# mit-acl/roman

Hardware: AMD Instinct MI355X
Metric: submap-pair alignments/sec + p50 latency at n=m=200 objects, d=512 (higher is better)
Workload: dtype f64 (fixed-point SpMV sums); 1 GPU; config 3: batch of 256 submap pairs per GPU, n=200 m=200 d=512, method=semanticgrav (xyz + 512-d descriptors + gravity prior); p50 latency measured on config 2 (single pair); pairs_per_call=256, n=200, m=200, d=512, method=semanticgrav, batches_in_flight=3

## Files before the change

### roman_amd/csrc/kernels.hip.h

```cpp
#pragma once
#include <hip/hip_cooperative_groups.h>
#include <hip/hip_runtime.h>
#include <stdint.h>
#include <type_traits>
#include "../../include/roman_hip.h"

namespace roman {

constexpr int WAVE = 64;
constexpr int STREAM_MAXL = 3072;

struct DevParams {
    roman_params_t p;
    double sig2;
    double sin_unc;
    double x_eps;
    double x_mindist;
    int32_t single;
    int32_t gravity;
    int32_t F;
    int32_t max_compact;
    int32_t gmode;
    int32_t diag_one;
    int32_t keep_all;
// ... 779 lines not shown
#pragma unroll
    for (int m = 0; m < MAXB; ++m) {
        if (m < cnt) {
            const int e = e0 + m, bx = e / nby, by = e - bx * nby;
            const int col = j0 + 16 * by + lr;
            const double nb = nrm[16 * T + 16 * by + lr];
#pragma unroll
            for (int r = 0; r < 4; ++r) {
                const int row = i0 + 16 * bx + kq + 4 * r;
                const double na = nrm[16 * bx + kq + 4 * r];
                if (row < iEnd && col < jEnd)
                    cosPool[pd.cosOff + (int64_t)row * pd.n2 + col] = D.pruned ? acc[m][r] : ((na > 0.0 && nb > 0.0) ? acc[m][r] / (na * nb) : 0.0);
            }
        }
    }
}

constexpr int CSEL_ROWS = 512;
constexpr int CSEL_MAXN = 256;
constexpr int CSEL_CAP = 4096;
constexpr int CSEL_NPT = CSEL_CAP / 1024;
constexpr int CSEL_P1 = 256 + 16;
constexpr int CSEL_P2 = 128 + 16;
constexpr int CSEL_MP = 11;
constexpr int CSEL_STAGE = CSEL_ROWS * CSEL_P1;
static_assert(CSEL_ROWS * CSEL_P2 + 2 * CSEL_CAP * 4 <= CSEL_STAGE, "pass 2 fits where the tile was");
constexpr int CSEL_LDS = CSEL_STAGE + CSEL_ROWS * 8 + 2 * 260 * 4;
typedef __bf16 bf16x8_t __attribute__((ext_vector_type(8)));
typedef float f32x4_t __attribute__((ext_vector_type(4)));
struct __attribute__((packed, aligned(8))) d8u_t { double v[8]; };

__device__ __forceinline__ bool csel_unsafe(double n) { return !(n >= 0x1p-40 && n <= 0x1p40); }

__global__ void __launch_bounds__(1024) k_cos_sel(DevParams D, int B, const ProbDesc* __restrict__ probs, const double* __restrict__ feats,
                                                  double* __restrict__ cosPool, int32_t* __restrict__ dense ,
                                                  double thr )
{
    extern __shared__ __attribute__((aligned(16))) unsigned char smem[];
    unsigned char* stage = smem;
    double* nrm = reinterpret_cast<double*>(smem + CSEL_STAGE);
    uint32_t* U = reinterpret_cast<uint32_t*>(smem + CSEL_ROWS * CSEL_P2);
    uint32_t* S = U + CSEL_CAP;
    int* hist = reinterpret_cast<int*>(nrm + CSEL_ROWS);
    int* cur = hist + 260;
    const int b = blockIdx.x;
    if (b >= B) return;
    const ProbDesc pd = probs[b];
    const int tid = threadIdx.x, lane = tid & 63, w = uni_i(tid >> 6);
    const int n1 = pd.n1, n2 = pd.n2;
    if (n1 <= 0 || n2 <= 0) { if (tid == 0) dense[b] = 0; return; }
    const int nb1 = (n1 + 15) >> 4, nb2 = (n2 + 15) >> 4, RB = 16 * nb1, nblk = nb1 * nb2, rowsTot = RB + 16 * nb2;
    if (n1 > CSEL_MAXN || n2 > CSEL_MAXN || nblk > 16 * CSEL_MP) { if (tid == 0) dense[b] = 1; return; }
    const int Fc = D.p.cos_feature_dim, coff = D.p.point_dim + D.p.ratio_feature_dim;
    if (tid < 260) hist[tid] = 0;
    const double* base1 = feats + pd.off1 * D.F + coff;
    const double* base2 = feats + pd.off2 * D.F + coff;

    constexpr int KT = 128, G1 = 4;
    const int nt = rowsTot >> 4;
    const int NG8 = ((nt + 2 * G1 - 1) / (2 * G1)) * 2;
    const int NSF = Fc / KT;
    uint32_t slotLo, slotHi;
    {
        const int R = w + 16 * min(lane, nt - 1);
        const bool isA = R < RB;
        const int idx = min(isA ? R : R - RB, (isA ? n1 : n2) - 1);
        const uint64_t pa = reinterpret_cast<uint64_t>((isA ? base1 : base2) + (int64_t)idx * D.F);
        slotLo = (uint32_t)pa; slotHi = (uint32_t)(pa >> 32);
    }
    auto slot_ptr = [&](int t) -> const double* {
        const uint64_t lo = (uint32_t)__builtin_amdgcn_readlane((int)slotLo, t), hi = (uint32_t)__builtin_amdgcn_readlane((int)slotHi, t);
        return reinterpret_cast<const double*>((hi << 32) | lo);
    };
    auto load_group = [&](dbl2_t (&x)[G1], int st, int g) {
        const int ko = st * KT + 2 * lane;
#pragma unroll
        for (int j = 0; j < G1; ++j) {
            const d2u_t tv = *reinterpret_cast<const d2u_t*>(slot_ptr(G1 * g + j) + ko);
            x[j] = dbl2_t{tv.v[0], tv.v[1]};
        }
        __builtin_amdgcn_sched_barrier(0);
    };
    auto load_group_ragged = [&](dbl2_t (&x)[G1], int st, int g) {
// ... 45 lines not shown
            }
        }
    };
    {
        dbl2_t xa[G1], xb[G1];
        if (NSF > 0) { load_group(xa, 0, 0); load_group(xb, 0, 1); }
        for (int st = 0; st < NSF; ++st) {
            for (int g = 0; g < NG8; g += 2) {
                const int gn = g + 2 < NG8 ? g + 2 : 0, stn = g + 2 < NG8 ? st : min(st + 1, NSF - 1);
                stage_group(xa, g);
                load_group(xa, stn, gn);
                stage_group(xb, g + 1);
                load_group(xb, stn, gn + 1);
            }
            __syncthreads();
            multiply();
            __syncthreads();
        }
        if (NSF * KT < Fc) {
            for (int g = 0; g < NG8; ++g) { load_group_ragged(xa, NSF, g); stage_group(xa, g); }
            __syncthreads();
            multiply();
            __syncthreads();
        }
    }
#pragma unroll
    for (int m = 0; m < 2; ++m)
        if (w + 16 * m < nt) {
            const int r4 = lane & 3;
            const float v = r4 == 0 ? accD[m][0] : r4 == 1 ? accD[m][1] : r4 == 2 ? accD[m][2] : accD[m][3];
            if (((lane & 15) >> 2) == (lane >> 4)) nrm[16 * (w + 16 * m) + (lane & 15)] = sqrt((double)v);
        }
    __syncthreads();

    const unsigned long long lt = (1ull << lane) - 1ull;
#pragma unroll
    for (int m = 0; m < CSEL_MP; ++m)
        if (m < cntP) {
            const int e = e0 + m, bx = e / nb2, by = e - bx * nb2;
            const int j = 16 * by + (lane & 15);
            const double nbv = nrm[RB + j];
#pragma unroll
            for (int rr = 0; rr < 4; ++rr) {
                const int i = 16 * bx + 4 * (lane >> 4) + rr;
                const double na = nrm[i];
                const bool ok = i < n1 && j < n2;
                const double cv = (double)acc[m][rr] / (na * nbv);
                const bool cand = ok && (csel_unsafe(na) || csel_unsafe(nbv) || !(cv < thr));
                if (ok && !cand) cosPool[pd.cosOff + (int64_t)i * n2 + j] = cv;
                const unsigned long long bm = __ballot(cand);
                if (bm) {
                    int base = 0;
                    if (lane == 0) base = atomicAdd(&hist[256], __popcll(bm));
                    base = __shfl(base, 0);
                    if (cand) {
                        const int slot = base + __popcll(bm & lt);
                        if (slot < CSEL_CAP) U[slot] = (uint32_t)i | ((uint32_t)j << 16);
                        atomicAdd(&hist[i], 1);
                    }
                }
            }
        }
    __syncthreads();
    const int nc = hist[256];
    if (nc > CSEL_CAP) { if (tid == 0) dense[b] = 1; return; }
    if (tid == 0) dense[b] = 0;
    if (nc == 0) return;
    if (w == 0) {
        const int c0 = hist[4 * lane], c1 = hist[4 * lane + 1], c2 = hist[4 * lane + 2], c3 = hist[4 * lane + 3];
        int incl = c0 + c1 + c2 + c3;
#pragma unroll
        for (int d = 1; d < 64; d <<= 1) { const int t = __shfl_up(incl, d); if (lane >= d) incl += t; }
        const int ex = incl - (c0 + c1 + c2 + c3);
        cur[4 * lane] = ex; cur[4 * lane + 1] = ex + c0; cur[4 * lane + 2] = ex + c0 + c1; cur[4 * lane + 3] = ex + c0 + c1 + c2;
    }
    __syncthreads();
    for (int q = tid; q < nc; q += 1024) { const uint32_t v = U[q]; S[atomicAdd(&cur[v & 0xffffu], 1)] = v; }
    __syncthreads();

    constexpr int NQ = CSEL_ROWS / 128;
    const int pp = lane & 7, laneRow = 8 * w + (lane >> 3);
    uint32_t rofs[NQ];
#pragma unroll
    for (int q = 0; q < NQ; ++q) {
        const int R = min(128 * q + laneRow, rowsTot - 1);
        const bool isA = R < RB;
        const int idx = min(isA ? R : R - RB, (isA ? n1 : n2) - 1);
        rofs[q] = (uint32_t)((((isA ? pd.off1 : pd.off2) + idx) * D.F + coff + 2 * pp) * 8);
    }
    const char* pool = reinterpret_cast<const char*>(feats);
    auto load16 = [&](dbl2_t (&x)[NQ], int k0) {
#pragma unroll
        for (int q = 0; q < NQ; ++q) { const d2u_t t = *reinterpret_cast<const d2u_t*>(pool + (rofs[q] + (uint32_t)(8 * k0))); x[q] = dbl2_t{t.v[0], t.v[1]}; }
    };
    auto load16_ragged = [&](dbl2_t (&x)[NQ], int k0) {
        const int k = k0 + 2 * pp;
#pragma unroll
        for (int q = 0; q < NQ; ++q) { const double* rb = reinterpret_cast<const double*>(pool + rofs[q]); x[q] = dbl2_t{k < Fc ? rb[k0] : 0.0, k + 1 < Fc ? rb[k0 + 1] : 0.0}; }
    };
    uint32_t my[CSEL_NPT]; double dot[CSEL_NPT];
    const int cnt2 = nc > tid ? (nc - tid + 1023) >> 10 : 0;
#pragma unroll
    for (int m = 0; m < CSEL_NPT; ++m) { my[m] = m < cnt2 ? S[m * 1024 + tid] : 0u; dot[m] = 0.0; }
    const int rN = tid >> 1, hN = tid & 1;
    double s0 = 0.0, s1 = 0.0;
    auto put16 = [&](const dbl2_t (&x)[NQ]) {
#pragma unroll
        for (int q = 0; q < NQ; ++q)
            *reinterpret_cast<dbl2_t*>(stage + (128 * q + laneRow) * CSEL_P2 + 16 * pp) = x[q];
    };
    auto compute = [&](int s, auto fullChunk) {
// ... 26 lines not shown
#pragma unroll
                        for (int g = 0; g < 4; ++g) if (4 * g + 2 * tp + 1 < kleft) d = fma(av[g].y, bv[g].y, d);
                    }
                }
                dot[m] = d;
            }
    };
    {
        const int NCF = Fc >> 4;
        dbl2_t ya[NQ], yb[NQ];
        if (NCF > 0) { load16(ya, 0); load16(yb, 16 * min(1, NCF - 1)); }
        for (int s = 0; s < NCF; s += 2) {
            put16(ya);
            __syncthreads();
            load16(ya, 16 * min(s + 2, NCF - 1));
            compute(s, std::true_type{});
            __syncthreads();
            if (s + 1 < NCF) {
                put16(yb);
                __syncthreads();
                load16(yb, 16 * min(s + 3, NCF - 1));
                compute(s + 1, std::true_type{});
                __syncthreads();
            }
        }
        if (NCF * 16 < Fc) {
            load16_ragged(ya, 16 * NCF);
            put16(ya);
            __syncthreads();
            compute(NCF, std::false_type{});
            __syncthreads();
        }
    }
    {
        const double p = s0 + s1, q = __shfl_xor(p, 1);
        if (hN == 0) nrm[rN] = sqrt(p + q);
    }
    __syncthreads();
#pragma unroll
    for (int m = 0; m < CSEL_NPT; ++m)
        if (m < cnt2) {
            const int i = (int)(my[m] & 0xffffu), j = (int)(my[m] >> 16);
            const double na = nrm[i], nbv = nrm[RB + j];
            cosPool[pd.cosOff + (int64_t)i * n2 + j] = (na > 0.0 && nbv > 0.0) ? dot[m] / (na * nbv) : 0.0;
        }
}

__global__ void __launch_bounds__(1024) k_tables(DevParams D, const ProbDesc* __restrict__ probs,
                                                 const double* __restrict__ feats,
                                                 double* __restrict__ tabPool, int RB ,
                                                 uint16_t* __restrict__ qtabPool )
{
    extern __shared__ __attribute__((aligned(16))) double s_xyz[];
    const ProbDesc pd = probs[blockIdx.z];
    const int which = blockIdx.y;
    const int n = which == 0 ? pd.n1 : pd.n2;
    const int r0 = blockIdx.x * RB;
    if (r0 >= n) return;
    const int64_t base = which == 0 ? pd.off1 : pd.off2;
    const int pdim = D.p.point_dim;
    for (int t = threadIdx.x; t < n * 3; t += blockDim.x) {
        const int o = t / 3, c = t - o * 3;
        s_xyz[t] = (c < pdim) ? feats[(base + o) * D.F + c] : 0.0;
    }
    __syncthreads();
    double* tab = tabPool + pd.tabOff + (which == 0 ? 0 : (int64_t)pd.n1 * pd.n1);
    const int nq = (n + 3) & ~3;
    uint16_t* qtab = qtabPool ? qtabPool + 4 * (int64_t)pd.qtabOff4 + (which == 0 ? 0 : (int64_t)pd.n1 * ((pd.n1 + 3) & ~3)) : nullptr;
    const int lane = threadIdx.x & 63, w = threadIdx.x >> 6, nw = blockDim.x >> 6;
    for (int rr = w; rr < RB; rr += nw) {
        const int a = r0 + rr;
        if (a >= n) break;
        const double ax = s_xyz[3 * a], ay = s_xyz[3 * a + 1], az = s_xyz[3 * a + 2];
        for (int b = lane; b < n; b += WAVE) {
            const double dx = ax - s_xyz[3 * b], dy = ay - s_xyz[3 * b + 1], dz = az - s_xyz[3 * b + 2];
            const double h2 = dx * dx + dy * dy;
            const double l2 = h2 + dz * dz;
            const bool bad = (a == b) || (D.p.mindist > 0.0 && l2 < D.x_mindist);
            const double v = (D.gmode == 1 || D.gmode == 2) ? sqrt(h2) : sqrt(l2);
            tab[(int64_t)a * n + b] = bad ? d_nan() : v;
            if (qtab) qtab[(int64_t)a * nq + b] = (uint16_t)(uint32_t)__builtin_fmin((bad ? d_nan() : v) * D.pre_invw, 32767.0);
        }
    }
}

constexpr int LIVE_CHUNK = 4096;

template <int PHASE>
__global__ void __launch_bounds__(256) k_live(DevParams D, const ProbDesc* __restrict__ probs,
                                              ProbState* __restrict__ st,
                                              const double* __restrict__ feats,
                                              const int32_t* __restrict__ assoc,
                                              const double* __restrict__ cosPool,
                                              double* __restrict__ qS, int32_t* __restrict__ qP ,
                                              int32_t* __restrict__ segCnt, int maxChunks,
                                              int32_t* __restrict__ lp, int32_t* __restrict__ li,
                                              int32_t* __restrict__ lj, double* __restrict__ ls, double* __restrict__ ld,
                                              double* __restrict__ lza, double* __restrict__ lzb)
{
    __shared__ int cbase[2];
    __shared__ uint16_t survQ[PHASE == 0 ? 4 : 1][PHASE == 0 ? LIVE_CHUNK / 4 : 1];
    const int b = blockIdx.y, c = blockIdx.x;
    const ProbDesc pd = probs[b];
    const int tid = threadIdx.x, w = tid >> 6, lane = tid & 63;
    const int nA = pd.nA;
    const int nChunks = (nA + LIVE_CHUNK - 1) / LIVE_CHUNK;
    if (c >= nChunks && !(PHASE == 1 && c == 0)) return;
    constexpr int SEG = LIVE_CHUNK / 4;
    constexpr int NIT = SEG / WAVE;
    const int p_beg = min(nA, c * LIVE_CHUNK + w * SEG), p_end = min(nA, p_beg + SEG);
    const int Fc = D.p.cos_feature_dim;
    const int64_t lo = pd.liveOff;
    int32_t* sc = segCnt + (int64_t)b * maxChunks * 4;
    const unsigned long long lt = (1ull << lane) - 1ull;

    if (PHASE == 0) {
        const int pdm = D.p.point_dim;
        auto full_score = [&](int p) {
            int i, j;
            decode_assoc(pd, assoc, p, i, j);
            const double cosv = (Fc > 0) ? cosPool[pd.cosOff + (int64_t)i * pd.n2 + j] : 0.0;
            const double* fi = feats + (pd.off1 + i) * D.F + pdm; const double* fj = feats + (pd.off2 + j) * D.F + pdm;
            return single_score(D, [&](int f) { return fi[f]; }, [&](int f) { return fj[f]; }, cosv);
        };
        int nlive = 0;
        auto emit = [&](bool valid, int p, double s) {
            const bool live = valid && (s > 0.0 || D.keep_all);
            const unsigned long long m = __ballot(live);
            if (live) { const int k = p_beg + nlive + __popcll(m & lt); qP[lo + k] = p; qS[lo + k] = s; }
            nlive += __popcll(m);
        };
        if (D.single && Fc > 0 && !D.keep_all) {
            uint16_t* q = survQ[w];
            const double cden = D.p.cosine_max - D.p.cosine_min;
            int ns = 0;
// ... 20 lines not shown
            __builtin_amdgcn_wave_barrier();
            __builtin_amdgcn_fence(__ATOMIC_ACQUIRE, "wavefront");
            for (int k0 = 0; k0 < ns; k0 += WAVE) {
                const int k = k0 + lane;
                const int p = p_beg + (int)q[min(k, max(ns - 1, 0))];
                emit(k < ns, p, k < ns ? full_score(p) : 0.0);
            }
        } else {
            for (int p0 = p_beg; p0 < p_end; p0 += WAVE) {
                const int p = p0 + lane;
                emit(p < p_end, p, (p < p_end && D.single) ? full_score(p) : 1.0);
            }
        }
        if (lane == 0) sc[c * 4 + w] = nlive;
        return;
    }

    if (w == 0) {
        int front = 0, total = 0;
        for (int k0 = 0; k0 < nChunks * 4; k0 += WAVE) {
            const int k = k0 + lane;
            const int v = k < nChunks * 4 ? sc[k] : 0;
            int f = k < c * 4 ? v : 0, t = v;
            for (int off = 32; off > 0; off >>= 1) { f += __shfl_xor(f, off); t += __shfl_xor(t, off); }
            front += f; total += t;
        }
        if (lane == 0) { cbase[0] = front; cbase[1] = total; }
    }
    __syncthreads();
    const bool all_live = D.pruned && cbase[1] == 0 && nA > 0;
    const int Ltot = all_live ? nA : cbase[1];
    if (c == 0 && tid == 0) {
        st[b].L = Ltot; st[b].nnzUpper = 0ull;
        st[b].kind = (Ltot <= D.stream_maxL && D.p.maxiniters >= 1 && D.p.maxlsiters >= 1) ? 0 : (D.allow_fallback ? 1 : 2);
    }
    if (c >= nChunks) return;
    int base = cbase[0];
    for (int k = 0; k < w; ++k) base += sc[c * 4 + k];
    const int n = all_live ? p_end - p_beg : sc[c * 4 + w];
    if (all_live) base = p_beg;
    const bool has_z = D.p.point_dim == 3;
    for (int k0 = 0; k0 < n; k0 += WAVE) {
        const int k = k0 + lane;
        if (k < n) {
            const int p = all_live ? p_beg + k : qP[lo + p_beg + k];
            const double s = all_live ? 1.0 : qS[lo + p_beg + k];
            int i, j;
            decode_assoc(pd, assoc, p, i, j);
            const int pos = base + k;
            lp[lo + pos] = p; li[lo + pos] = i; lj[lo + pos] = j; ls[lo + pos] = s;
            ld[lo + pos] = D.diag_one ? 1.0 : s;
            lza[lo + pos] = has_z ? feats[(pd.off1 + i) * D.F + 2] : 0.0;
            lzb[lo + pos] = has_z ? feats[(pd.off2 + j) * D.F + 2] : 0.0;
        }
    }
}

template <class T>
__device__ __forceinline__ T block_excl_scan(T v, T* sh, T& total)
{
    const int lane = threadIdx.x & 63, w = threadIdx.x >> 6, nw = blockDim.x >> 6;
    T inc = v;
    for (int off = 1; off < WAVE; off <<= 1) { const T t = __shfl_up(inc, off); if (lane >= off) inc += t; }
    __syncthreads();
    if (lane == WAVE - 1) sh[w] = inc;
    __syncthreads();
    T base = 0, tot = 0;
// ... 4374 lines not shown
```

### roman_amd/csrc/roman_hip.hip

```cpp
#include <hip/hip_runtime.h>
#include <algorithm>
#include <cmath>
#include <cstdarg>
#include <cstdio>
#include <cstdlib>
#include <cstring>
#include <new>
#include <string>
#include <vector>

#include "kernels.hip.h"

using namespace roman;

namespace {

thread_local std::string g_last_error;

struct DevBuf {
    void* p = nullptr; size_t cap = 0;
    hipError_t ensure(size_t bytes) {
        if (bytes <= cap) return hipSuccess;
        if (p) { hipError_t e = hipFree(p); p = nullptr; cap = 0; if (e != hipSuccess) return e; }
        size_t want = bytes + bytes / 4 + 256;
// ... 269 lines not shown
        heurMaxL = std::max(heurMaxL, (int)capL);
        heurMask += capL * std::ceil(capL / 64.0);
        heurNnz += capL * std::min(capL, 96.0);
    }
    if (H.valid) {
        S->expectMaxL = prunes ? (int)std::min(S->maxA, std::ceil(H.rMaxL * S->maxA * 1.15) + 64.0) : (int)S->maxA;
        S->capMaskWords = (long long)(prunes ? H.rMask * S->maskBound * 1.3 + 4096.0 : S->maskBound);
        S->capNnz = (long long)(H.rNnz * S->sumA * 1.3 + 65536.0);
        S->capList = (long long)(H.rList * S->sumA * 1.3 + 65536.0);
    } else {
        S->expectMaxL = heurMaxL; S->capMaskWords = (long long)heurMask; S->capNnz = (long long)heurNnz + 65536;
        S->capList = (long long)(2.5 * heurNnz) + 65536;
    }
    S->capMaskWords = std::max<long long>(S->capMaskWords, 64);
    const char* tcap = getenv("ROMAN_TEST_CAPNNZ");
    if (tcap && !H.valid) S->capNnz = atoll(tcap);
}

int may_fallback(const DevParams& D, const std::vector<ProbDesc>& hd);

struct BatchOut { int32_t kmax; int32_t* assoc_out; int32_t* n_assoc_out; double* T_out; int32_t* status_out; roman_stats_t* stats_out; };

int make_solve_out(roman_ctx* c, int B, int64_t sumA, const BatchOut& out, SolveOut* O)
{
    const size_t R1 = (size_t)std::max<int64_t>(sumA, 1);
    HIPCHK(c, WS.uOut.ensure(sizeof(double) * R1)); HIPCHK(c, WS.nodesOrig.ensure(sizeof(int32_t) * R1));
    HIPCHK(c, WS.nSel.ensure(sizeof(int32_t) * (size_t)B));
    O->assoc_out = out.assoc_out; O->n_assoc_out = out.n_assoc_out; O->T_out = out.T_out; O->status_out = out.status_out; O->stats_out = out.stats_out; O->kmax = out.kmax;
    O->nodesOrig = WS.nodesOrig.as<int32_t>(); O->nSel = WS.nSel.as<int32_t>(); O->uOut = WS.uOut.as<double>();
    O->dbg = nullptr;
    return ROMAN_OK;
}

static hipError_t launch_cos_sel(roman_ctx* c, hipStream_t stream, const DevParams& D, int B, int maxN1, int maxN2, const ProbDesc* dP, const double* feats, double* cosPool,
                                 int32_t* dense, bool approx)
{
    hipError_t e = dyn_lds(c, reinterpret_cast<const void*>(k_cos_sel), (size_t)CSEL_LDS);
    if (e != hipSuccess) return e;
    const double thr = approx ? INFINITY : D.p.cosine_min - 0x1p-6;
    hipLaunchKernelGGL(k_cos_sel, dim3((unsigned)B), dim3(1024), (size_t)CSEL_LDS, stream, D, B, dP, feats, cosPool, dense, thr);
    e = hipGetLastError();
    if (e != hipSuccess) return e;
    constexpr int TD = 5;
    using CD = CosDeal<TD>;
    const int Gd = CD::tiles(maxN1) * CD::tiles(maxN2);
    e = dyn_lds(c, reinterpret_cast<const void*>(k_cos_deal<TD, 0>), (size_t)CD::LDS);
    if (e != hipSuccess) return e;
    hipLaunchKernelGGL((k_cos_deal<TD, 0>), dim3((unsigned)(B >= 8 ? Gd * ((B + 7) / 8) * 8 : Gd * B)), dim3(256), (size_t)CD::LDS, stream, D, B, Gd, dP, feats, cosPool, (const int32_t*)dense);
    return hipGetLastError();
}
static bool cos_sel_applies(const roman_ctx* c, const DevParams& D, int B, int maxN1, int maxN2, int64_t poolRows)
{
    if (!D.single || D.pruned || !(D.p.cosine_max > D.p.cosine_min) || !std::isfinite(D.p.cosine_min) || !std::isfinite(D.p.cosine_max)) return false;
    if (maxN1 > CSEL_MAXN || maxN2 > CSEL_MAXN || maxN1 <= 0 || maxN2 <= 0) return false;
    if (poolRows * (int64_t)D.F * 8 >= (1LL << 32)) return false;
    const char* env = getenv("ROMAN_COS_SEL");
    if (env && env[0]) return env[0] == '1';
    if (2 * B < c->num_cu || D.p.cos_feature_dim < 64 || std::max(maxN1, maxN2) < 64) return false;
    roman_ctx::Hist& H = const_cast<roman_ctx*>(c)->hist;
    if (H.cosSeen && H.cosDenseFrac > 0.25) {
        if (++H.cosSkipped < 64) return false;
        H.cosSkipped = 0;
    }
    return true;
}


static int sort_eq_max()
{
    const char* e = getenv("ROMAN_SORT_EQMAX");
    return (e && e[0]) ? std::max(0, atoi(e)) : 512;
}

static hipError_t launch_cos(roman_ctx* c, hipStream_t stream, const DevParams& D, int B, int maxN1, int maxN2, const ProbDesc* dP, const double* feats, double* cosPool)
{
// ... 26 lines not shown
        const int nbx = (maxN1 + 15) / 16, nby = (maxN2 + 15) / 16;
        if (!(blockEnv && blockEnv[0] == '0') && (int64_t)B * nbx * nby <= 8 * (int64_t)c->num_cu) {
            hipLaunchKernelGGL(k_cos_block, dim3((unsigned)((B * nbx * nby + 3) / 4)), dim3(256), 0, stream, D, B, nbx, nby, dP, feats, cosPool);
            return hipGetLastError();
        }
    }
    if (mode == 0) {
        const int tiles = ((maxN1 + COS_TILE - 1) / COS_TILE) * ((maxN2 + COS_TILE - 1) / COS_TILE), G = (tiles + 3) / 4;
        hipLaunchKernelGGL(k_cos, dim3((unsigned)(G * ((B + 7) / 8) * 8)), dim3(256), 0, stream, D, B, G, dP, feats, cosPool);
        return hipGetLastError();
    }
    auto tiles = [](int n) { return (((n + 15) >> 4) + 3) >> 2; };
    const int G = tiles(maxN1) * tiles(maxN2);
    const int KC = mode == 32 ? 32 : 16;
    const size_t lds = (size_t)2 * 128 * (KC * 8 + 16);
    auto kf = KC == 16 ? k_cos_tile<16> : k_cos_tile<32>;
    const hipError_t e = dyn_lds(c, reinterpret_cast<const void*>(kf), lds);
    if (e != hipSuccess) return e;
    static const char* wgEnv = getenv("ROMAN_COS_WGS");
    const int perCu = wgEnv ? atoi(wgEnv) : 0;
    const int total = G * ((B + 7) / 8) * 8;
    const int grid = perCu > 0 ? std::min(total, (c->num_cu & ~7) * perCu) : total;
    hipLaunchKernelGGL(kf, dim3((unsigned)grid), dim3(256), lds, stream, D, B, G, dP, feats, cosPool);
    return hipGetLastError();
}

int enqueue_score(roman_ctx* c, const DevParams& Din, const roman_params_t* params, const BatchIn& in, std::vector<ProbDesc>& hd, DevParams* Dout,
                  const BatchOut* smallOut = nullptr, const double* smallU0 = nullptr)
{
    const int B = in.B;
    hd.assign(B, ProbDesc{});
    int64_t sumA = 0, sumCos = 0, sumTab = 0, sumQ4 = 0;
    int maxN12 = 0, maxN = 0, maxA = 0, maxN1 = 0, maxN2 = 0; int64_t maxTab = 0, poolRows = 0 ;
    for (int b = 0; b < B; ++b) {
        ProbDesc& d = hd[b];
        d.off1 = in.off1[b]; d.off2 = in.off2[b]; d.n1 = in.n1[b]; d.n2 = in.n2[b];
        if (d.n1 < 0 || d.n2 < 0) return fail(c, ROMAN_E_INVALID, "negative map size in problem %d", b);
        const int64_t na_list = in.assoc ? in.assoc_off[b + 1] - in.assoc_off[b] : 0;
        if (in.assoc && (na_list < 0 || na_list > 2147483647LL || in.assoc_off[b] < 0)) return fail(c, ROMAN_E_INVALID, "bad assoc_off at problem %d", b);
        if (in.assoc && na_list > 0) {
            d.assocOff = in.assoc_off[b];
            d.nA = (int32_t)na_list;
        } else {
            d.assocOff = -1;
            const int64_t na = (int64_t)d.n1 * d.n2;
            if (na > 2147483647LL) return fail(c, ROMAN_E_TOO_LARGE, "n1*n2 overflows int32 in problem %d", b);
            d.nA = (int32_t)na;
        }
        d.liveOff = sumA; d.cosOff = sumCos; d.tabOff = sumTab; d.normOff = 0;
        if (sumQ4 > 2147483647LL) return fail(c, ROMAN_E_TOO_LARGE, "the tables of this batch exceed the bin pool's 32-bit offsets; split it");
        d.qtabOff4 = (int32_t)sumQ4;
        sumQ4 += ((int64_t)d.n1 * ((d.n1 + 3) & ~3) + (int64_t)d.n2 * ((d.n2 + 3) & ~3)) / 4;
        maxA = std::max(maxA, d.nA);
        sumA += d.nA; sumCos += (int64_t)d.n1 * d.n2; sumTab += (int64_t)d.n1 * d.n1 + (int64_t)d.n2 * d.n2;
        maxN12 = std::max(maxN12, d.n1 + d.n2); maxN = std::max(maxN, std::max(d.n1, d.n2));
        maxN1 = std::max(maxN1, d.n1); maxN2 = std::max(maxN2, d.n2);
        maxTab = std::max(maxTab, (int64_t)d.n1 * d.n1 + (int64_t)d.n2 * d.n2);
        poolRows = std::max(poolRows, std::max(d.off1 + d.n1, d.off2 + d.n2));
    }
    if (sumA > 2000000000LL) return fail(c, ROMAN_E_TOO_LARGE, "batch has %lld associations; split it (limit 2e9 per call)", (long long)sumA);
    const size_t nA1 = (size_t)std::max<int64_t>(sumA, 1);
    DevParams D = Din;
    const bool cosOn = D.p.cos_feature_dim > 0;

    Sizing SZ;
    estimate_sizes(c, D, params, in.F, hd, &SZ);
    SZ.capMaskWords = std::max(SZ.capMaskWords, WS.capMaskWords); SZ.capNnz = std::max(SZ.capNnz, WS.capNnz); SZ.capList = std::max(SZ.capList, WS.capList);
    D.stream_maxL = std::min(STREAM_MAXL, std::max(64, (SZ.expectMaxL + 63) & ~63));
    { static const char* smEnv = getenv("ROMAN_STREAM_MAXL"); if (smEnv) D.stream_maxL = std::max(64, std::min(D.stream_maxL, atoi(smEnv))); }
    D.allow_fallback = (!c->hist.valid || SZ.expectMaxL > D.stream_maxL || D.p.maxiniters < 1 || D.p.maxlsiters < 1) ? 1 : 0;
    {
        static const char* wideEnv = getenv("ROMAN_WIDE");
        const int mayFb = may_fallback(D, hd);
        const bool bigLiveSets = !(D.single && !D.keep_all) || c->hist.valid;
        D.wide = (c->coop_ok && mayFb > 0 && D.p.maxiniters >= 1 && D.p.maxlsiters >= 1 && maxA <= (int64_t)WIDE_KW * c->num_cu * WIDE_NW * 64 &&
// ... 20 lines not shown
    HIPCHK(c, WS.listPool.ensure(sizeof(uint16_t) * (size_t)std::max<long long>(SZ.capList, 4)));
    HIPCHK(c, WS.prefPool.ensure(sizeof(uint32_t) * (size_t)SZ.capMaskWords));
    HIPCHK(c, WS.vals.ensure(sizeof(double) * (size_t)SZ.capNnz));
    HIPCHK(c, WS.cols16.ensure(sizeof(uint16_t) * (size_t)SZ.capNnz));
    HIPCHK(c, WS.cols32.ensure(sizeof(uint32_t) * (size_t)SZ.capNnz));
    WS.capMaskWords = SZ.capMaskWords; WS.capNnz = SZ.capNnz; WS.capList = SZ.capList;
    int RPB = 32;
    while (RPB < 128 && (int64_t)RPB * c->num_cu * 64 < sumA) RPB <<= 1;
    { const char* e_ = getenv("ROMAN_RPB"); if (e_ && e_[0]) { const int v_ = atoi(e_); if (v_ == 32 || v_ == 64 || v_ == 128) RPB = v_; } }
    const size_t maxItems = (size_t)(sumA / RPB) + (size_t)B + 1;
    HIPCHK(c, WS.items.ensure(sizeof(ItemDesc) * maxItems));

    {
        if (WS.probsPending) { HIPCHK(c, hipEventSynchronize(WS.probsEvent)); WS.probsPending = false; }
        if (WS.pinnedProbsCap < (size_t)B) {
            if (WS.pinnedProbs) (void)hipHostFree(WS.pinnedProbs);
            WS.pinnedProbs = nullptr; WS.pinnedProbsCap = 0;
            const size_t cap = std::max<size_t>((size_t)B * 2, 64);
            HIPCHK(c, hipHostMalloc((void**)&WS.pinnedProbs, sizeof(ProbDesc) * cap, hipHostMallocDefault));
            WS.pinnedProbsCap = cap;
        }
        memcpy(WS.pinnedProbs, hd.data(), sizeof(ProbDesc) * (size_t)B);
        HIPCHK(c, hipMemcpyAsync(WS.probs.p, WS.pinnedProbs, sizeof(ProbDesc) * (size_t)B, hipMemcpyHostToDevice, WS.stream));
        HIPCHK(c, hipEventRecord(WS.probsEvent, WS.stream));
        WS.probsPending = true;
    }
    const ProbDesc* dP = WS.probs.as<ProbDesc>();
    ProbState* dS = WS.state.as<ProbState>();
    BatchTotals* dT = WS.totals.as<BatchTotals>();
    const LivePools LP{WS.lp.as<int32_t>(), WS.li.as<int32_t>(), WS.lj.as<int32_t>(), WS.ls.as<double>(), WS.ld.as<double>(), WS.lza.as<double>(), WS.lzb.as<double>()};
    const LivePools PP{WS.plp.as<int32_t>(), WS.pli.as<int32_t>(), WS.plj.as<int32_t>(), WS.pls.as<double>(), WS.pld.as<double>(), WS.plza.as<double>(), WS.plzb.as<double>()};

    StageTimer t0(c, ROMAN_STAGE_SINGLE);
    bool cosScreen = false;
    if (cosOn && maxN1 > 0 && maxN2 > 0) {
        cosScreen = cos_sel_applies(c, D, B, maxN1, maxN2, poolRows);
        ++(cosScreen ? c->cosScreenBatches : c->cosDenseBatches);
        if (cosScreen) {
            HIPCHK(c, WS.cosDense.ensure(sizeof(int32_t) * (size_t)B));
            HIPCHK(c, launch_cos_sel(c, WS.stream, D, B, maxN1, maxN2, dP, in.feats, WS.cosPool.as<double>(), WS.cosDense.as<int32_t>(), false));
        } else
        HIPCHK(c, launch_cos(c, WS.stream, D, B, maxN1, maxN2, dP, in.feats, WS.cosPool.as<double>()));
    DBG(c, "k_cos");
    }
    if (maxTab > 0) {
        const size_t tabLds = sizeof(double) * 3 * (size_t)std::max(maxN, 1);
        if (tabLds > c->lds_max) return fail(c, ROMAN_E_TOO_LARGE, "maps of %d objects exceed the LDS point staging of this build", maxN);
        HIPCHK(c, dyn_lds(c, reinterpret_cast<const void*>(k_tables), tabLds));
        const int bands = std::max(1, std::min((maxN + 15) / 16, (2 * c->num_cu + 2 * B - 1) / (2 * B)));
        const int RBt = (((maxN + bands - 1) / bands) + 15) & ~15;
        const int thr = RBt >= 64 ? 1024 : 256;
        uint16_t* qtab = nullptr;
        if (D.pre_invw > 0.0 && std::isfinite(D.pre_invw)) {
            HIPCHK(c, WS.qtabPool.ensure(sizeof(uint16_t) * 4 * (size_t)std::max<int64_t>(sumQ4, 1) + 64));
            qtab = WS.qtabPool.as<uint16_t>();
        }
        hipLaunchKernelGGL(k_tables, dim3((unsigned)((maxN + RBt - 1) / RBt), 2, B), dim3(thr), tabLds, WS.stream, D, dP, in.feats, WS.tabPool.as<double>(), RBt, qtab);
    DBG(c, "k_tables");
    }
    {
        const int maxChunks = std::max(1, (maxA + LIVE_CHUNK - 1) / LIVE_CHUNK);
        HIPCHK(c, WS.chunkCnt.ensure(sizeof(int32_t) * (size_t)B * (size_t)maxChunks * 4));
        hipLaunchKernelGGL(k_live<0>, dim3((unsigned)maxChunks, (unsigned)B), dim3(256), 0, WS.stream, D, dP, dS, in.feats, in.assoc, WS.cosPool.as<double>(), WS.sTmp.as<double>(), PP.lp ,
                           WS.chunkCnt.as<int32_t>(), maxChunks, LP.lp, LP.li, LP.lj, LP.ls, LP.ld, LP.lza, LP.lzb);
        hipLaunchKernelGGL(k_live<1>, dim3((unsigned)maxChunks, (unsigned)B), dim3(256), 0, WS.stream, D, dP, dS, in.feats, in.assoc, WS.cosPool.as<double>(), WS.sTmp.as<double>(), PP.lp ,
                           WS.chunkCnt.as<int32_t>(), maxChunks, LP.lp, LP.li, LP.lj, LP.ls, LP.ld, LP.lza, LP.lzb);
    DBG(c, "k_live");
    }
    t0.stop();

    const int expL = std::max(SZ.expectMaxL, 1);
    const int ldsPerRow = ((2 * std::max(maxN, 1) + 1 + 1) & ~1) + 2;
    const int colBytesC = D.gravity ? 20 : 4;
    const int Lneed = (expL + 255) & ~255;
    int NRc = ((size_t)16 * 2 * ldsPerRow * sizeof(double) + (size_t)std::min(Lneed, 2048) * colBytesC <= c->lds_max) ? 2 : 1;
    int wpb = 16;
    static const char* nrEnv = getenv("ROMAN_COUNT_NR");
    static const char* wpbEnv = getenv("ROMAN_COUNT_WPB");
    if (nrEnv) NRc = atoi(nrEnv) == 2 ? 2 : 1;
    if (wpbEnv) wpb = std::max(1, std::min(16, atoi(wpbEnv)));
    while (wpb > 1 && (size_t)wpb * NRc * ldsPerRow * sizeof(double) + 256 * colBytesC > c->lds_max) wpb >>= 1;
    if ((size_t)wpb * NRc * ldsPerRow * sizeof(double) + 256 * colBytesC > c->lds_max)
        return fail(c, ROMAN_E_TOO_LARGE, "maps of %d objects exceed the LDS table staging of this build", maxN);
    const int ldsPerWave = NRc * ldsPerRow;
    const size_t tabLds = (size_t)wpb * ldsPerWave * sizeof(double);
    int TCc = (int)std::min<size_t>((c->lds_max - tabLds) / colBytesC, 32768) & ~255;
    TCc = std::min(TCc, Lneed);
    const size_t pairLds = tabLds + (size_t)TCc * colBytesC;
    const int pairGrid = c->num_cu * std::max(1, std::min(2048 / (wpb * 64), (int)(c->lds_max / pairLds)));
    int preNR = 0, preWpb = 0, preTC = 0, preNO = 0; size_t preLds = 0;
    const int preRow = (2 * std::max(maxN, 1) + 1 + 3) & ~3;
    {
        const char* preEnv = getenv("ROMAN_COUNT_PRE");
        const bool want = (preEnv ? preEnv[0] != '0' : true) && D.pre_invw > 0.0 && std::isfinite(D.pre_invw) && Lneed <= (preEnv ? 16000 : 4096) && maxN <= 32767;
        if (want) {
            const int tc = Lneed;
            for (int wp = PRE_WAVES; wp >= 8; wp -= 4) {
                const size_t need = (size_t)(tc + PRE_COLPAD + 4) * 4 + (size_t)wp * (size_t)count_pre_wave_bytes(preRow, tc);
                if (need <= c->lds_max) { preNR = PRE_NR; preWpb = wp; preTC = tc; preLds = need; break; }
// ... 1427 lines not shown
```

Before: 168,300 alignments/s.

## Fuse live-pair scoring and compaction into the cosine screening kernel

Adds a LIVE variant of the cosine screening kernel. For all-to-all problems without keep_all, it computes single scores for candidate pairs inside the screening kernel, builds a per-row live bitmap in LDS and writes the compacted live pools and problem state directly. This skips the cosPool writes and lets the two k_live passes exit early for problems the fused kernel handled, removing a global round trip of n1*n2 cosines and two passes of chunk scanning. In exchange the screening kernel's tail does more serial work (score evaluation, a prefix scan and scattered writes), and problems flagged dense still go through the old path.

```diff
diff --git a/roman_amd/csrc/kernels.hip.h b/roman_amd/csrc/kernels.hip.h
--- a/roman_amd/csrc/kernels.hip.h
+++ b/roman_amd/csrc/kernels.hip.h
@@ -835,9 +835,16 @@
 
 __device__ __forceinline__ bool csel_unsafe(double n) { return !(n >= 0x1p-40 && n <= 0x1p40); }
 
-__global__ void __launch_bounds__(1024) k_cos_sel(DevParams D, int B, const ProbDesc* __restrict__ probs, const double* __restrict__ feats,
-                                                  double* __restrict__ cosPool, int32_t* __restrict__ dense ,
-                                                  double thr )
+__device__ __forceinline__ int live_kind(const DevParams& D, int L)
+{
+    return (L <= D.stream_maxL && D.p.maxiniters >= 1 && D.p.maxlsiters >= 1) ? 0 : (D.allow_fallback ? 1 : 2);
+}
+
+struct CselLive { ProbState* st; int32_t* lp; int32_t* li; int32_t* lj; double* ls; double* ld; double* lza; double* lzb; };
+
+template <bool LIVE>
+__device__ __forceinline__ void cos_sel_body(const DevParams& D, int B, const ProbDesc* __restrict__ probs, const double* __restrict__ feats,
+                                             double* __restrict__ cosPool, int32_t* __restrict__ dense, double thr, const CselLive& lv)
 {
     extern __shared__ __attribute__((aligned(16))) unsigned char smem[];
     unsigned char* stage = smem;
@@ -851,7 +858,16 @@
     const ProbDesc pd = probs[b];
     const int tid = threadIdx.x, lane = tid & 63, w = uni_i(tid >> 6);
     const int n1 = pd.n1, n2 = pd.n2;
-    if (n1 <= 0 || n2 <= 0) { if (tid == 0) dense[b] = 0; return; }
+    auto publish = [&](int L) {
+        if (LIVE && tid == 0) { lv.st[b].L = L; lv.st[b].nnzUpper = 0ull; lv.st[b].kind = live_kind(D, L); }
+    };
+#ifdef ROMAN_CSEL_TIMING
+    unsigned long long tc_[5]; tc_[0] = __builtin_readcyclecounter();
+#define CMARK(i_) tc_[i_] = __builtin_readcyclecounter()
+#else
+#define CMARK(i_) do { } while (0)
+#endif
+    if (n1 <= 0 || n2 <= 0) { if (tid == 0) dense[b] = 0; publish(0); return; }
     const int nb1 = (n1 + 15) >> 4, nb2 = (n2 + 15) >> 4, RB = 16 * nb1, nblk = nb1 * nb2, rowsTot = RB + 16 * nb2;
     if (n1 > CSEL_MAXN || n2 > CSEL_MAXN || nblk > 16 * CSEL_MP) { if (tid == 0) dense[b] = 1; return; }
     const int Fc = D.p.cos_feature_dim, coff = D.p.point_dim + D.p.ratio_feature_dim;
@@ -963,6 +979,7 @@
             if (((lane & 15) >> 2) == (lane >> 4)) nrm[16 * (w + 16 * m) + (lane & 15)] = sqrt((double)v);
         }
     __syncthreads();
+    CMARK(1);
 
     const unsigned long long lt = (1ull << lane) - 1ull;
 #pragma unroll
@@ -978,7 +995,7 @@
                 const bool ok = i < n1 && j < n2;
                 const double cv = (double)acc[m][rr] / (na * nbv);
                 const bool cand = ok && (csel_unsafe(na) || csel_unsafe(nbv) || !(cv < thr));
-                if (ok && !cand) cosPool[pd.cosOff + (int64_t)i * n2 + j] = cv;
+                if (!LIVE && ok && !cand) cosPool[pd.cosOff + (int64_t)i * n2 + j] = cv;
                 const unsigned long long bm = __ballot(cand);
                 if (bm) {
                     int base = 0;
@@ -996,7 +1013,7 @@
     const int nc = hist[256];
     if (nc > CSEL_CAP) { if (tid == 0) dense[b] = 1; return; }
     if (tid == 0) dense[b] = 0;
-    if (nc == 0) return;
+    if (nc == 0) { publish(0); return; }
     if (w == 0) {
         const int c0 = hist[4 * lane], c1 = hist[4 * lane + 1], c2 = hist[4 * lane + 2], c3 = hist[4 * lane + 3];
         int incl = c0 + c1 + c2 + c3;
@@ -1008,6 +1025,7 @@
     __syncthreads();
     for (int q = tid; q < nc; q += 1024) { const uint32_t v = U[q]; S[atomicAdd(&cur[v & 0xffffu], 1)] = v; }
     __syncthreads();
+    CMARK(2);
 
     constexpr int NQ = CSEL_ROWS / 128;
     const int pp = lane & 7, laneRow = 8 * w + (lane >> 3);
@@ -1100,18 +1118,90 @@
             __syncthreads();
         }
     }
+    CMARK(3);
+    unsigned long long* liveBits = reinterpret_cast<unsigned long long*>(stage);
+    static_assert(CSEL_MAXN * (CSEL_MAXN / 64) <= 1024 && CSEL_MAXN * (CSEL_MAXN / 64) * 8 <= CSEL_ROWS * CSEL_P2, "one word per thread, in pass 2's chunk");
+    if (LIVE) liveBits[tid] = 0ull;
     {
         const double p = s0 + s1, q = __shfl_xor(p, 1);
         if (hN == 0) nrm[rN] = sqrt(p + q);
     }
     __syncthreads();
-#pragma unroll
-    for (int m = 0; m < CSEL_NPT; ++m)
+    double sc[CSEL_NPT];
+    bool live[CSEL_NPT];
+#pragma unroll
+    for (int m = 0; m < CSEL_NPT; ++m) {
+        live[m] = false; sc[m] = 0.0;
         if (m < cnt2) {
             const int i = (int)(my[m] & 0xffffu), j = (int)(my[m] >> 16);
             const double na = nrm[i], nbv = nrm[RB + j];
-            cosPool[pd.cosOff + (int64_t)i * n2 + j] = (na > 0.0 && nbv > 0.0) ? dot[m] / (na * nbv) : 0.0;
-        }
+            const double cosv = (na > 0.0 && nbv > 0.0) ? dot[m] / (na * nbv) : 0.0;
+            if (!LIVE) cosPool[pd.cosOff + (int64_t)i * n2 + j] = cosv;
+            else if ((cosv - D.p.cosine_min) / (D.p.cosine_max - D.p.cosine_min) > 0.0) {
+                const int pdm = D.p.point_dim;
+                const double* fi = feats + (pd.off1 + i) * D.F + pdm; const double* fj = feats + (pd.off2 + j) * D.F + pdm;
+                sc[m] = single_score(D, [&](int f) { return fi[f]; }, [&](int f) { return fj[f]; }, cosv);
+                live[m] = sc[m] > 0.0;
+                if (live[m]) atomicOr(&liveBits[4 * i + (j >> 6)], 1ull << (j & 63));
+            }
+        }
+    }
+    if (!LIVE) { CMARK(4); }
+    else {
+        __syncthreads();
+        if (w == 0) {
+            int c4[4];
+#pragma unroll
+            for (int k = 0; k < 4; ++k) {
+                const unsigned long long* rw = liveBits + 4 * (4 * lane + k);
+                c4[k] = __popcll(rw[0]) + __popcll(rw[1]) + __popcll(rw[2]) + __popcll(rw[3]);
+            }
+            int incl = c4[0] + c4[1] + c4[2] + c4[3];
+#pragma unroll
+            for (int d = 1; d < 64; d <<= 1) { const int t = __shfl_up(incl, d); if (lane >= d) incl += t; }
+            const int ex = incl - (c4[0] + c4[1] + c4[2] + c4[3]);
+            cur[4 * lane] = ex; cur[4 * lane + 1] = ex + c4[0]; cur[4 * lane + 2] = ex + c4[0] + c4[1]; cur[4 * lane + 3] = ex + c4[0] + c4[1] + c4[2];
+            if (lane == 63) cur[256] = incl;
+        }
+        __syncthreads();
+        const int64_t lo = pd.liveOff;
+        const bool has_z = D.p.point_dim == 3;
+#pragma unroll
+        for (int m = 0; m < CSEL_NPT; ++m)
+            if (live[m]) {
+                const int i = (int)(my[m] & 0xffffu), j = (int)(my[m] >> 16), wj = j >> 6;
+                const unsigned long long* rw = liveBits + 4 * i;
+                int pos = cur[i] + __popcll(rw[wj] & ((1ull << (j & 63)) - 1ull));
+                for (int k = 0; k < wj; ++k) pos += __popcll(rw[k]);
+                const double s = sc[m];
+                lv.lp[lo + pos] = i * n2 + j; lv.li[lo + pos] = i; lv.lj[lo + pos] = j; lv.ls[lo + pos] = s;
+                lv.ld[lo + pos] = D.diag_one ? 1.0 : s;
+                lv.lza[lo + pos] = has_z ? feats[(pd.off1 + i) * D.F + 2] : 0.0;
+                lv.lzb[lo + pos] = has_z ? feats[(pd.off2 + j) * D.F + 2] : 0.0;
+            }
+        publish(cur[256]);
+        CMARK(4);
+    }
+#ifdef ROMAN_CSEL_TIMING
+    if (tid == 0 && (b & 63) == 0) printf("[%s] b=%d candidates=%d cycles: pass1 %llu select %llu pass2 %llu tail %llu\n", LIVE ? "k_cos_live" : "k_cos_sel", b, nc,
+                                          tc_[1] - tc_[0], tc_[2] - tc_[1], tc_[3] - tc_[2], tc_[4] - tc_[3]);
+#endif
+#undef CMARK
+}
+
+__global__ void __launch_bounds__(1024) k_cos_sel(DevParams D, int B, const ProbDesc* __restrict__ probs, const double* __restrict__ feats,
+                                                  double* __restrict__ cosPool, int32_t* __restrict__ dense ,
+                                                  double thr )
+{
+    cos_sel_body<false>(D, B, probs, feats, cosPool, dense, thr, CselLive{});
+}
+
+__global__ void __launch_bounds__(1024) k_cos_live(DevParams D, int B, const ProbDesc* __restrict__ probs, const double* __restrict__ feats,
+                                                   int32_t* __restrict__ dense , double thr ,
+                                                   ProbState* __restrict__ st, int32_t* __restrict__ lp, int32_t* __restrict__ li, int32_t* __restrict__ lj,
+                                                   double* __restrict__ ls, double* __restrict__ ld, double* __restrict__ lza, double* __restrict__ lzb)
+{
+    cos_sel_body<true>(D, B, probs, feats, nullptr, dense, thr, CselLive{st, lp, li, lj, ls, ld, lza, lzb});
 }
 
 __global__ void __launch_bounds__(1024) k_tables(DevParams D, const ProbDesc* __restrict__ probs,
@@ -1164,11 +1254,13 @@
                                               int32_t* __restrict__ segCnt, int maxChunks,
                                               int32_t* __restrict__ lp, int32_t* __restrict__ li,
                                               int32_t* __restrict__ lj, double* __restrict__ ls, double* __restrict__ ld,
-                                              double* __restrict__ lza, double* __restrict__ lzb)
+                                              double* __restrict__ lza, double* __restrict__ lzb,
+                                              const int32_t* __restrict__ only )
 {
     __shared__ int cbase[2];
     __shared__ uint16_t survQ[PHASE == 0 ? 4 : 1][PHASE == 0 ? LIVE_CHUNK / 4 : 1];
     const int b = blockIdx.y, c = blockIdx.x;
+    if (only && !only[b]) return;
     const ProbDesc pd = probs[b];
     const int tid = threadIdx.x, w = tid >> 6, lane = tid & 63;
     const int nA = pd.nA;
@@ -1255,7 +1347,7 @@
     const int Ltot = all_live ? nA : cbase[1];
     if (c == 0 && tid == 0) {
         st[b].L = Ltot; st[b].nnzUpper = 0ull;
-        st[b].kind = (Ltot <= D.stream_maxL && D.p.maxiniters >= 1 && D.p.maxlsiters >= 1) ? 0 : (D.allow_fallback ? 1 : 2);
+        st[b].kind = live_kind(D, Ltot);
     }
     if (c >= nChunks) return;
     int base = cbase[0];
diff --git a/roman_amd/csrc/roman_hip.hip b/roman_amd/csrc/roman_hip.hip
--- a/roman_amd/csrc/roman_hip.hip
+++ b/roman_amd/csrc/roman_hip.hip
@@ -325,6 +325,8 @@
     return ROMAN_OK;
 }
 
+static hipError_t launch_cos_flagged(roman_ctx* c, hipStream_t stream, const DevParams& D, int B, int maxN1, int maxN2, const ProbDesc* dP, const double* feats,
+                                     double* cosPool, const int32_t* dense);
 static hipError_t launch_cos_sel(roman_ctx* c, hipStream_t stream, const DevParams& D, int B, int maxN1, int maxN2, const ProbDesc* dP, const double* feats, double* cosPool,
                                  int32_t* dense, bool approx)
 {
@@ -334,6 +336,23 @@
     hipLaunchKernelGGL(k_cos_sel, dim3((unsigned)B), dim3(1024), (size_t)CSEL_LDS, stream, D, B, dP, feats, cosPool, dense, thr);
     e = hipGetLastError();
     if (e != hipSuccess) return e;
+    return launch_cos_flagged(c, stream, D, B, maxN1, maxN2, dP, feats, cosPool, dense);
+}
+static hipError_t launch_cos_live(roman_ctx* c, hipStream_t stream, const DevParams& D, int B, int maxN1, int maxN2, const ProbDesc* dP, const double* feats, double* cosPool,
+                                  int32_t* dense, ProbState* st, const LivePools& LP)
+{
+    hipError_t e = dyn_lds(c, reinterpret_cast<const void*>(k_cos_live), (size_t)CSEL_LDS);
+    if (e != hipSuccess) return e;
+    hipLaunchKernelGGL(k_cos_live, dim3((unsigned)B), dim3(1024), (size_t)CSEL_LDS, stream, D, B, dP, feats, dense, D.p.cosine_min - 0x1p-6,
+                       st, LP.lp, LP.li, LP.lj, LP.ls, LP.ld, LP.lza, LP.lzb);
+    e = hipGetLastError();
+    if (e != hipSuccess) return e;
+    return launch_cos_flagged(c, stream, D, B, maxN1, maxN2, dP, feats, cosPool, dense);
+}
+static hipError_t launch_cos_flagged(roman_ctx* c, hipStream_t stream, const DevParams& D, int B, int maxN1, int maxN2, const ProbDesc* dP, const double* feats,
+                                     double* cosPool, const int32_t* dense)
+{
+    hipError_t e;
     constexpr int TD = 5;
     using CD = CosDeal<TD>;
     const int Gd = CD::tiles(maxN1) * CD::tiles(maxN2);
@@ -426,6 +445,7 @@
     hd.assign(B, ProbDesc{});
     int64_t sumA = 0, sumCos = 0, sumTab = 0, sumQ4 = 0;
     int maxN12 = 0, maxN = 0, maxA = 0, maxN1 = 0, maxN2 = 0; int64_t maxTab = 0, poolRows = 0 ;
+    bool allToAll = true;
     for (int b = 0; b < B; ++b) {
         ProbDesc& d = hd[b];
         d.off1 = in.off1[b]; d.off2 = in.off2[b]; d.n1 = in.n1[b]; d.n2 = in.n2[b];
@@ -435,6 +455,7 @@
         if (in.assoc && na_list > 0) {
             d.assocOff = in.assoc_off[b];
             d.nA = (int32_t)na_list;
+            allToAll = false;
         } else {
             d.assocOff = -1;
             const int64_t na = (int64_t)d.n1 * d.n2;
@@ -521,13 +542,17 @@
     const LivePools PP{WS.plp.as<int32_t>(), WS.pli.as<int32_t>(), WS.plj.as<int32_t>(), WS.pls.as<double>(), WS.pld.as<double>(), WS.plza.as<double>(), WS.plzb.as<double>()};
 
     StageTimer t0(c, ROMAN_STAGE_SINGLE);
-    bool cosScreen = false;
+    bool cosScreen = false, cosLive = false;
     if (cosOn && maxN1 > 0 && maxN2 > 0) {
         cosScreen = cos_sel_applies(c, D, B, maxN1, maxN2, poolRows);
         ++(cosScreen ? c->cosScreenBatches : c->cosDenseBatches);
         if (cosScreen) {
             HIPCHK(c, WS.cosDense.ensure(sizeof(int32_t) * (size_t)B));
-            HIPCHK(c, launch_cos_sel(c, WS.stream, D, B, maxN1, maxN2, dP, in.feats, WS.cosPool.as<double>(), WS.cosDense.as<int32_t>(), false));
+            cosLive = allToAll && !D.keep_all;
+            if (cosLive)
+                HIPCHK(c, launch_cos_live(c, WS.stream, D, B, maxN1, maxN2, dP, in.feats, WS.cosPool.as<double>(), WS.cosDense.as<int32_t>(), dS, LP));
+            else
+                HIPCHK(c, launch_cos_sel(c, WS.stream, D, B, maxN1, maxN2, dP, in.feats, WS.cosPool.as<double>(), WS.cosDense.as<int32_t>(), false));
         } else
         HIPCHK(c, launch_cos(c, WS.stream, D, B, maxN1, maxN2, dP, in.feats, WS.cosPool.as<double>()));
     DBG(c, "k_cos");
@@ -549,11 +574,12 @@
     }
     {
         const int maxChunks = std::max(1, (maxA + LIVE_CHUNK - 1) / LIVE_CHUNK);
+        const int32_t* only = cosLive ? WS.cosDense.as<int32_t>() : nullptr;
         HIPCHK(c, WS.chunkCnt.ensure(sizeof(int32_t) * (size_t)B * (size_t)maxChunks * 4));
         hipLaunchKernelGGL(k_live<0>, dim3((unsigned)maxChunks, (unsigned)B), dim3(256), 0, WS.stream, D, dP, dS, in.feats, in.assoc, WS.cosPool.as<double>(), WS.sTmp.as<double>(), PP.lp ,
-                           WS.chunkCnt.as<int32_t>(), maxChunks, LP.lp, LP.li, LP.lj, LP.ls, LP.ld, LP.lza, LP.lzb);
+                           WS.chunkCnt.as<int32_t>(), maxChunks, LP.lp, LP.li, LP.lj, LP.ls, LP.ld, LP.lza, LP.lzb, only);
         hipLaunchKernelGGL(k_live<1>, dim3((unsigned)maxChunks, (unsigned)B), dim3(256), 0, WS.stream, D, dP, dS, in.feats, in.assoc, WS.cosPool.as<double>(), WS.sTmp.as<double>(), PP.lp ,
-                           WS.chunkCnt.as<int32_t>(), maxChunks, LP.lp, LP.li, LP.lj, LP.ls, LP.ld, LP.lza, LP.lzb);
+                           WS.chunkCnt.as<int32_t>(), maxChunks, LP.lp, LP.li, LP.lj, LP.ls, LP.ld, LP.lza, LP.lzb, only);
     DBG(c, "k_live");
     }
     t0.stop();
```

Result: faster. 173,600 alignments/s (median of 6 runs) (+3.1%).
